# LPD-EPFL-ML/X-MAP

Hardware: NVIDIA B200
Metric: item_pair_sims_per_sec (higher is better)
Workload: dtype f64 epilogue over i64 fixed-point accumulators

## Files before the change

### include/xmap_b200.h

```cpp
#ifndef XMAP_B200_H
#define XMAP_B200_H

#include <stdbool.h>
#include <stddef.h>
#include <stdint.h>

#ifdef __cplusplus
extern "C" {
#endif

#define XMAP_B200_ABI_VERSION 8
#define XMAP_KMAX 64
#define XMAP_METHOD_ADJUST_COSINE 0
#define XMAP_METHOD_COSINE 1

int xmap_abi_version(void);
const char *xmap_last_error(void);

size_t xmap_layout_workspace_bytes(int64_t nnz, int32_t n_users, int32_t n_items);

int xmap_build_layout(const int32_t *user, const int32_t *item, const float *rating,
                      int64_t nnz, int32_t n_users, int32_t n_items,
                      int32_t *csr_ptr, uint64_t *csr_ent, int32_t *csr_src,
                      int32_t *csc_ptr, uint64_t *csc_ent,
                      double *user_mu, double *item_stats,
                      void *workspace, size_t workspace_bytes, void *stream);

int xmap_row_work(const int32_t *csr_ptr, const int32_t *csc_ptr, const uint64_t *csc_ent,
                  int32_t n_items, int64_t *row_work, void *stream);

size_t xmap_tri_workspace_bytes(int64_t nnz);
int xmap_build_tri_layout(const int32_t *csr_ptr, const uint64_t *csr_ent,
                          const int32_t *csc_ptr, const uint64_t *csc_ent,
                          const double *user_mu, const double *item_stats, const int32_t *prefix_code,
                          const int32_t *ord, int32_t n_users, int32_t n_items, int64_t nnz, int32_t method,
                          int32_t e_base, uint64_t *tcsr_ent, void *csc_aux, void *ostat, int64_t *tri_work,
                          void *workspace, size_t workspace_bytes, void *stream);

typedef struct xmap_sim_args {
    const int32_t *csc_ptr; const uint64_t *csc_ent; const void *csc_aux;
    const uint64_t *tcsr_ent;
    const void *ostat; const int32_t *ord; const int64_t *tri_work;
    const int32_t *ord_item;
    const uint8_t *dom_code;
    const uint8_t *contains;
    int32_t n_items; int32_t method; int32_t num_atleast; int32_t k;
    int32_t r2_bits;
    int32_t count_only;
    const int64_t *rec_ptr;
    int32_t *rec_cnt;
    void *rec;
    int32_t *rec_n;
    uint8_t *bb;
    int32_t *row_npairs;
    int32_t *tab_idx; double *tab_sim; int32_t *tab_mutu; int32_t *tab_n; int32_t *tab_len;
    int32_t *error_flag;
} xmap_sim_args;

#define XMAP_SIM_ROW_HDR_BYTES 48
int xmap_sim_row_headers(const xmap_sim_args *args_h, const int32_t *rows, int32_t n_rows,
                         const int32_t *seg_lo, const int32_t *seg_hi, void *hdr_out, void *stream);

#define XMAP_SIM_MAX_SMEM_CELLS 12288
int64_t xmap_sim_row_cells(int64_t tri_work, int32_t n_more_popular);
int xmap_sim_accumulate(const xmap_sim_args *args_h, const void *row_hdr, int32_t n_rows,
                        int32_t cells_cap, int32_t threads_per_row,
                        void *gtab, int32_t gtab_ctas, void *stream);

int xmap_sim_accumulate_split(const xmap_sim_args *args_h, const void *seg_hdr, const int32_t *seg_slot,
                              const int32_t *slot_nseg, int32_t n_segs, int32_t cells_cap, void *gtab,
                              int32_t *done, void *stream);

#define XMAP_SELECT_LONG 8192
int xmap_sim_select(const xmap_sim_args *args_h, const int32_t *rows, int32_t n_rows,
                    int32_t long_rows, void *stream);

int xmap_segmented_copy16(const void *src, const int64_t *src_pos, void *dst, const int64_t *dst_pos,
                          const int64_t *seg_off, int32_t n_seg, int64_t total, void *stream);
int xmap_segmented_copy4(const void *src, const int64_t *src_pos, void *dst, const int64_t *dst_pos,
                         const int64_t *seg_off, int32_t n_seg, int64_t total, void *stream);

#define XMAP_XSIM_MAX_CELLS_LG 13
typedef struct xmap_xsim_args {
    int32_t n_starts;
    int32_t n_units;
    const int32_t *unit_order;
    int32_t *unit_counter;
    int32_t warps;
    const int64_t *unit_leg_lo, *unit_leg_hi;
    const int32_t *unit_g0, *unit_g1;
    const int32_t *unit_npass;
    const int32_t *start_unit_ptr;
    const int64_t *lp_ptr;
    const int32_t *pd_s;
    const double *pd_n, *pd_d, *pd_c;
    const int64_t *rs_ptr;
    const int32_t *rs_end;
    const double *rs_n, *rs_d, *rs_c;
    const int32_t *tile_ptr; int32_t gb;
    int32_t cells_lg;
    const int32_t *unit_clg;
    void *gws; int32_t gcells_lg;
    int32_t top_m;
    int32_t merge;
    int32_t *unit_count; int64_t *unit_combos;
    int32_t *unit_top_end; double *unit_top_xsim; int32_t *unit_top_len;
    int32_t *out_count; int64_t *out_combos;
    int32_t *top_end; double *top_xsim; int32_t *top_len;
    const int64_t *emit_ptr; int32_t *emit_end; double *emit_xsim;
    int32_t *error_flag;
    int64_t *unit_cycles;
} xmap_xsim_args;

int64_t xmap_xsim_smem_bytes(int32_t cells_lg, int32_t warps);
int xmap_xsim_extend(const xmap_xsim_args *args_h, void *stream);
int64_t xmap_xsim_cta_smem_bytes(int32_t cells_lg);
int xmap_xsim_extend_cta(const xmap_xsim_args *args_h, void *stream);
int xmap_xsim_merge(const xmap_xsim_args *args_h, void *stream);

int xmap_choose_mapping(const int32_t *top_end, const double *top_xsim, const int32_t *top_len,
                        int32_t n_rows, int32_t top_m, int32_t mode, int32_t n_cand,
                        double epsilon, int32_t mapping_range, int32_t global_sensitivity,
                        const double *uniforms, uint64_t seed,
                        int32_t *chosen, void *stream);

int xmap_invert_mapping(const int32_t *start_item, const int32_t *chosen, int32_t n_rows,
                        int32_t *map, void *stream);

size_t xmap_alterego_workspace_bytes(int64_t nnz);
int xmap_build_alterego(const int32_t *csr_ptr, const uint64_t *csr_ent, const int32_t *csr_src,
                        const int64_t *ts, int32_t n_users, int64_t nnz, const int32_t *map,
                        int32_t *out_user, int32_t *out_item, double *out_rating, int64_t *out_ts,
                        int64_t *n_out_h, void *workspace, size_t workspace_bytes, void *stream);

int xmap_recsim_item_info(const int64_t *item_ptr, const double *rating_by_item, int32_t n_items, double *info,
                          void *stream);
int xmap_recsim_fill_entries(const int64_t *user_ptr, const int64_t *ent_off, int32_t n_users, const int32_t *item,
                             int64_t n_items, int64_t total, int64_t *key, int64_t *src, void *stream);
int xmap_recsim_pairs(const int64_t *seg_ptr, const int64_t *seg_key, const int64_t *src, const double *rating,
                      const double *info, int64_t n_items, int64_t n_pairs, int32_t num_atleast,
                      int32_t *out_i, int32_t *out_j, int64_t *out_n, double *out_sim, double *out_ls, void *stream);

int xmap_recsim_neighbors(const int64_t *row_ptr, const int32_t *pair_j, const double *pair_sim, int32_t n_items,
                          int32_t k, int32_t *nb_idx, double *nb_sim, int32_t *nb_len, void *stream);
int xmap_recsim_predict(const int64_t *prof_ptr, const int32_t *prof_item, const double *prof_rating,
                        const int64_t *prof_ts, const double *info, const int32_t *nb_idx, const double *nb_sim,
                        const int32_t *nb_len, int32_t k, const int32_t *t_user, const int32_t *t_item, int64_t n_test,
                        double alpha, double *pred_nodecay, double *pred_decay, int32_t *error_flag, void *stream);

int xmap_recsim_private_neighbor(const int64_t *row_ptr, const int32_t *nbr, const double *sim, const double *ls,
                                 int32_t n_items, int32_t mapping_range, double eps, double rpo,
                                 const double *u_pick, const double *u_noise, uint64_t seed, double *scratch,
                                 int32_t *out_nbr, double *out_sim, int32_t *out_len, void *stream);

int xmap_clean_records(const int32_t *user, const int32_t *item, const double *ts, const int64_t *order,
                       int64_t n, int32_t n_users, double t_lo, double t_hi, int32_t num_atleast,
                       uint8_t *keep, int32_t *user_items, void *stream);

#define XMAP_INGEST_ID_MAX 48
#define XMAP_INGEST_OK 0
#define XMAP_INGEST_BLANK 1
#define XMAP_INGEST_FEW_FIELDS 2
#define XMAP_INGEST_NON_ASCII 3
#define XMAP_INGEST_NUL 4
#define XMAP_INGEST_BAD_TIME 5
#define XMAP_INGEST_TIME_RANGE 6
#define XMAP_INGEST_BAD_RATING 7
#define XMAP_INGEST_UID_LONG 8
#define XMAP_INGEST_IID_LONG 9
int xmap_ingest_line_masks(const void *buf, int64_t size, uint16_t *masks, int32_t *block_cnt, void *stream);
int xmap_ingest_line_offsets(const uint16_t *masks, int64_t size, const int64_t *block_off, int64_t *offs, void *stream);
int xmap_ingest_parse(const uint8_t *buf, const int64_t *offs, int64_t n_lines, const char *label_h, int32_t label_len,
                      double ts_min, double ts_max, int64_t ld, uint8_t *status, double *rating, double *ts,
                      uint64_t *uid_words, uint8_t *uid_len, uint64_t *iid_words, uint8_t *iid_len, void *stream);
int xmap_ingest_rank_flags(const uint64_t *words, int64_t ld, int32_t n_words, const int64_t *perm, int64_t n,
                           int32_t *flag, void *stream);
int xmap_ingest_rank_scatter(const int64_t *perm, const int32_t *flag, const int64_t *csum, int64_t n, int32_t *rank,
                             int64_t *rep, void *stream);
int xmap_ingest_first(const int32_t *user, const int32_t *item, const double *ts, const int64_t *order,
                      const uint8_t *keep, int64_t n, double t_lo, double t_hi, int32_t *first_user, int32_t *pair_first,
                      void *stream);
int xmap_ingest_item_suffix(const uint64_t *iid_words, int64_t ld, const uint8_t *iid_len, const int64_t *rep,
                            int32_t n_items, uint8_t *present, void *stream);
int xmap_ingest_item_codes(const uint64_t *iid_words, int64_t ld, const uint8_t *iid_len, const int64_t *rep,
                           int32_t n_items, const int32_t *labels, int32_t n_labels, int32_t *prefix_new,
                           uint8_t *dom_code, uint8_t *contains, bool *has_S, bool *has_T, void *stream);
int xmap_ingest_train_keys(const int32_t *user, const int32_t *item, const int8_t *grp, const int32_t *upos,
                           const bool *has_S, const int32_t *srank, int64_t n, int64_t *key, void *stream);

#ifdef __cplusplus
}
#endif
#endif
```

### x-map_b200/csrc/sim.cu

```cuda
#include "common.cuh"

namespace xmap {

constexpr int KMAX = XMAP_KMAX;

struct __align__(16) OStat {
    double den;
    uint32_t item;
    uint32_t prefix_exp;
};

struct __align__(16) Cell {
    unsigned key, cnt, lo, hi;
};

struct __align__(16) Rec {
    unsigned long long sim;
    unsigned long long pack;
};
__device__ __forceinline__ unsigned long long rec_pack(unsigned item, unsigned mutu) {
    return (unsigned long long)item | ((unsigned long long)mutu << 32);
}
__device__ __forceinline__ int rec_item(unsigned long long p) { return int((unsigned)p); }
__device__ __forceinline__ int rec_mutu(unsigned long long p) { return int((unsigned)(p >> 32)); }

struct __align__(16) RowHdr {
    int row, oi, lo, hi;
    long long work;
    double den;
    long long rec_base;
    unsigned prefix_exp;
    int rec_cap;
};
static_assert(sizeof(RowHdr) == 48, "RowHdr layout");

__device__ __forceinline__ RowHdr load_hdr(const RowHdr *p) {
    const uint4 *q = reinterpret_cast<const uint4 *>(p);
    const uint4 a = __ldg(q), b = __ldg(q + 1), c = __ldg(q + 2);
    RowHdr h;
    h.row = (int)a.x; h.oi = (int)a.y; h.lo = (int)a.z; h.hi = (int)a.w;
    h.work = (long long)(((unsigned long long)b.y << 32) | b.x);
    h.den = __hiloint2double((int)b.w, (int)b.z);
    h.rec_base = (long long)(((unsigned long long)c.y << 32) | c.x);
    h.prefix_exp = c.z; h.rec_cap = (int)c.w;
    return h;
}

__global__ void row_headers_kernel(xmap_sim_args a, const int32_t *__restrict__ rows, int n_rows,
                                   const int32_t *__restrict__ seg_lo, const int32_t *__restrict__ seg_hi,
                                   RowHdr *__restrict__ out) {
    const int r = blockIdx.x * blockDim.x + threadIdx.x;
    if (r >= n_rows) return;
    const int row = rows[r];
    const OStat *ostat = reinterpret_cast<const OStat *>(a.ostat);
    RowHdr h;
    h.row = row; h.oi = a.ord[row];
    h.lo = seg_lo ? seg_lo[r] : a.csc_ptr[row];
    h.hi = seg_hi ? seg_hi[r] : a.csc_ptr[row + 1];
    h.work = a.tri_work[row];
    const OStat si = ostat[h.oi];
    h.den = si.den; h.prefix_exp = si.prefix_exp;
    h.rec_base = a.rec_ptr[row];
    h.rec_cap = (int)(a.rec_ptr[row + 1] - a.rec_ptr[row]);
    out[r] = h;
}

__host__ __device__ __forceinline__ long long hash_cells_for(long long work) {
    long long c = (work * 4 + 2) / 3;
    return c < 32 ? 32 : c;
}

template <bool CTA_ROW>
__device__ __forceinline__ void group_sync() {
    if (CTA_ROW) __syncthreads(); else __syncwarp();
}

struct RaterDesc {
    unsigned start;
    int len;
    double ci, mu;
};

__device__ __forceinline__ RaterDesc load_rater(const xmap_sim_args &a, int e, int hi) {
    RaterDesc d{0u, 0, 0.0, 0.0};
    if (e < hi) {
        const uint2 ce = ld_ent(a.csc_ent + e);
        const uint4 ax = __ldg(reinterpret_cast<const uint4 *>(a.csc_aux) + e);
        d.mu = __hiloint2double((int)ax.w, (int)ax.z);
        d.ci = (double)__uint_as_float(ce.y) - d.mu;
        d.start = (ax.x + 1u) | (ce.x & 0x80000000u);
        d.len = (int)ax.y;
    }
    return d;
}

struct SplitCtx {
    uint4 *gtab;
    int *done;
    int nseg;
};

template <bool CTA_ROW, class IDX>
__device__ void tri_row(const xmap_sim_args &a, Cell *__restrict__ T, IDX *__restrict__ occ_list, int *s_cnt,
                        int cells_cap, const RowHdr *hdr_p, const SplitCtx *sp = nullptr) {
    const int lane = threadIdx.x & 31;
    const int gwarps = CTA_ROW ? (blockDim.x >> 5) : 1;
    const int gw = CTA_ROW ? (threadIdx.x >> 5) : 0;
    const int gthreads = gwarps * 32, gtid = gw * 32 + lane;
    const unsigned lt_mask = (1u << lane) - 1u;
    const OStat *__restrict__ ostat = reinterpret_cast<const OStat *>(a.ostat);

    const RowHdr hd = load_hdr(hdr_p);
    const int row = hd.row, oi = hd.oi;
    const int e_i = int(hd.prefix_exp & 0xFFu);
    const unsigned prefix_i = hd.prefix_exp >> 8;
    const int lo = hd.lo, hi = hd.hi;
    const long long work = hd.work;
    const int rtop = a.n_items - 1 - oi;
    const long long hcells = hash_cells_for(work);
    const bool direct = (long long)rtop <= hcells;
    const long long ncell_ll = direct ? (long long)rtop : hcells;
    if (ncell_ll > cells_cap || (!direct && min((long long)(hi - lo), work) >= 65536)) {
        if (gtid == 0) atomicExch(a.error_flag, ncell_ll > cells_cap ? 1 : 3);
        return;
    }
    const int ncell = (int)ncell_ll;
    uint4 *T4 = reinterpret_cast<uint4 *>(T);
    for (int s = gtid; s < ncell; s += gthreads) T4[s] = make_uint4(0u, 0u, 0u, 0u);
    if (CTA_ROW && gtid == 0) *s_cnt = 0;
    group_sync<CTA_ROW>();

    const int qbase = 62 - a.r2_bits;
    const int top_ord = a.n_items - 1;
    const bool coop = CTA_ROW && ((hi - lo + 31) >> 5) < gwarps;
    const int bfirst = coop ? 0 : gw, bstride = coop ? 1 : gwarps;
    const int cfirst = coop ? gw : 0, cstride = coop ? gwarps : 1;
    constexpr int UC = 2;
    RaterDesc nxt = load_rater(a, lo + bfirst * 32 + lane, hi);
    for (int b0 = lo + bfirst * 32; b0 < hi; b0 += bstride * 32) {
        const RaterDesc cur = nxt;
        nxt = load_rater(a, b0 + bstride * 32 + lane, hi);
        int incl = cur.len;
#pragma unroll
        for (int off = 1; off < 32; off <<= 1) {
            const int t = __shfl_up_sync(0xffffffffu, incl, off);
            if (lane >= off) incl += t;
        }
        const int total = __shfl_sync(0xffffffffu, incl, 31);
        const int excl = incl - cur.len;
        for (int t0 = cfirst * 32; t0 < total; t0 += cstride * 32 * UC) {
            uint2 en[UC];
            unsigned st_l[UC];
            double ci_l[UC], mu_l[UC];
            bool valid[UC];
#pragma unroll
            for (int u = 0; u < UC; ++u) {
                const int t = t0 + u * cstride * 32 + lane;
                int l = 0;
#pragma unroll
                for (int step = 16; step >= 1; step >>= 1) {
                    const int v = __shfl_sync(0xffffffffu, incl, l + step - 1);
                    if (v <= t) l += step;
                }
                st_l[u] = __shfl_sync(0xffffffffu, cur.start, l);
                const int ex_l = __shfl_sync(0xffffffffu, excl, l);
                ci_l[u] = __shfl_sync(0xffffffffu, cur.ci, l);
                mu_l[u] = __shfl_sync(0xffffffffu, cur.mu, l);
                valid[u] = t < total;
                if (valid[u]) en[u] = ld_ent(a.tcsr_ent + ((st_l[u] & 0x7FFFFFFFu) + (unsigned)(t - ex_l)));
            }
#pragma unroll
            for (int u = 0; u < UC; ++u) {
                if (!valid[u]) continue;
                const int oj = ent_item(en[u].x);
                const double cj = (double)__uint_as_float(en[u].y) - mu_l[u];
                const double p = __dmul_rn(ci_l[u], cj);
                const int q = qbase - (e_i + ent_exp(en[u].x));
                const long long fx = __double2ll_rn(p * pow2d(q));
                const unsigned agree = ((unsigned)ent_ge(en[u].x) == (st_l[u] >> 31)) ? 1u : 0u;
                int slot;
                bool ok = true;
                if (direct) {
                    slot = top_ord - oj;
                    atomicAdd(agree ? &T[slot].key : &T[slot].cnt, 1u);
                } else {
                    const unsigned key = (unsigned)oj + 1u;
                    slot = (int)__umulhi((unsigned)oj * 2654435761u, (unsigned)ncell);
                    ok = false;
                    for (int probe = 0; probe < ncell; ++probe) {
                        unsigned c = *(volatile unsigned *)&T[slot].key;
                        if (c != key) {
                            if (c == 0u) c = atomicCAS(&T[slot].key, 0u, key);
                            if (c != 0u && c != key) { slot = (slot + 1 == ncell) ? 0 : slot + 1; continue; }
                        }
                        ok = true;
                        break;
                    }
                    if (ok) atomicAdd(&T[slot].cnt, (1u << 16) | agree);
                    else atomicExch(a.error_flag, 1);
                }
                if (ok) {
                    if (sizeof(IDX) == 4) {
                        atomicAdd(reinterpret_cast<unsigned long long *>(&T[slot].lo), (unsigned long long)fx);
                    } else {
                        const unsigned flo = (unsigned)(unsigned long long)fx;
                        unsigned fhi = (unsigned)((unsigned long long)fx >> 32);
                        if (flo) {
                            const unsigned old = atomicAdd(&T[slot].lo, flo);
                            fhi += ((unsigned)(old + flo) < old) ? 1u : 0u;
                        }
                        if (fhi) atomicAdd(&T[slot].hi, fhi);
                    }
                }
            }
        }
    }
    group_sync<CTA_ROW>();

    if (CTA_ROW && sp) {
        if (!direct) {
            if (gtid == 0) atomicExch(a.error_flag, 1);
            return;
        }
        for (int s = gtid; s < ncell; s += gthreads) {
            const uint4 v = T4[s];
            if (v.x) atomicAdd(&sp->gtab[s].x, v.x);
            if (v.y) atomicAdd(&sp->gtab[s].y, v.y);
            const unsigned long long fx = ((unsigned long long)v.w << 32) | v.z;
            if (fx) atomicAdd(reinterpret_cast<unsigned long long *>(&sp->gtab[s].z), fx);
        }
        __threadfence();
        __syncthreads();
        if (gtid == 0) *s_cnt = (atomicAdd(sp->done, 1) == sp->nseg - 1) ? 1 : 0;
        __syncthreads();
        const bool last = *s_cnt != 0;
        __syncthreads();
        if (!last) return;
        __threadfence();
        for (int s = gtid; s < ncell; s += gthreads) {
            T4[s] = __ldcg(sp->gtab + s);
            sp->gtab[s] = make_uint4(0u, 0u, 0u, 0u);
        }
        if (gtid == 0) { *sp->done = 0; *s_cnt = 0; }
        __syncthreads();
    }

    int n_ent = 0;
    for (int s0 = gw * 32; s0 < ncell; s0 += gthreads) {
        const int s = s0 + lane;
        bool occ = false;
        if (s < ncell) {
            const uint2 kc = *reinterpret_cast<const uint2 *>(&T[s]);
            occ = direct ? (kc.x | kc.y) != 0u : kc.x != 0u;
        }
        const unsigned m = __ballot_sync(0xffffffffu, occ);
        if (m) {
            int base = n_ent;
            if (CTA_ROW) {
                if (lane == 0) base = atomicAdd(s_cnt, __popc(m));
                base = __shfl_sync(0xffffffffu, base, 0);
            }
            if (occ) occ_list[base + __popc(m & lt_mask)] = (IDX)s;
            n_ent += __popc(m);
        }
    }
    group_sync<CTA_ROW>();
    if (CTA_ROW) n_ent = *s_cnt;
    if (gtid == 0 && n_ent) a.row_npairs[row] += n_ent;

    constexpr int EU = 2;
    int nkept = 0;
    for (int i0 = gtid; i0 < n_ent; i0 += gthreads * EU) {
        uint4 cv[EU];
        int sidx[EU];
        unsigned n[EU], mutu[EU];
        OStat sj[EU];
#pragma unroll
        for (int u = 0; u < EU; ++u) {
            const int i = i0 + u * gthreads;
            sidx[u] = -1;
            if (i < n_ent) {
                sidx[u] = (int)occ_list[i];
                cv[u] = T4[sidx[u]];
                int oj;
                if (direct) { n[u] = cv[u].x + cv[u].y; mutu[u] = cv[u].x; oj = top_ord - sidx[u]; }
                else { oj = (int)cv[u].x - 1; n[u] = cv[u].y >> 16; mutu[u] = cv[u].y & 0xFFFFu; }
                sj[u] = ostat[oj];
            }
        }
#pragma unroll
        for (int u = 0; u < EU; ++u) {
            if (sidx[u] < 0) continue;
            uint4 out = make_uint4(0u, 0u, 0u, 0u);
            const int q = qbase - (e_i + int(sj[u].prefix_exp & 0xFFu));
            const long long fx = (long long)(((unsigned long long)cv[u].w << 32) | (unsigned long long)cv[u].z);
            if (fx == 0 || mutu[u] == 0u) { T4[sidx[u]] = out; continue; }
            const double inner = (double)fx * pow2d(-q);
            const double dd = __dmul_rn(hd.den, sj[u].den);
            const double cosv = (dd != 0.0) ? __ddiv_rn(inner, dd) : 0.0;
            const int mn = min((int)n[u], a.num_atleast);
            const double sim = __ddiv_rn(__dmul_rn(cosv, (double)mn), (double)a.num_atleast);
            if (sim != 0.0 && mutu[u] != 0u) {
                ++nkept;
                const unsigned long long sb = (unsigned long long)__double_as_longlong(sim);
                out = direct ? make_uint4(mutu[u], n[u], (unsigned)sb, (unsigned)(sb >> 32))
                             : make_uint4(sj[u].item, (n[u] << 16) | mutu[u], (unsigned)sb, (unsigned)(sb >> 32));
                if ((sj[u].prefix_exp >> 8) != prefix_i) { a.bb[row] = 1; a.bb[sj[u].item] = 1; }
            }
            T4[sidx[u]] = out;
        }
    }
#pragma unroll
    for (int off = 16; off > 0; off >>= 1) nkept += __shfl_xor_sync(0xffffffffu, nkept, off);
    if (nkept == 0) return;

    Rec *__restrict__ rec = reinterpret_cast<Rec *>(a.rec);
    const long long base_i = hd.rec_base;
    const int cap_i = hd.rec_cap;
    int wbase = 0;
    if (lane == 0) wbase = atomicAdd(a.rec_cnt + row, nkept);
    wbase = __shfl_sync(0xffffffffu, wbase, 0);
    if (a.count_only) {
        for (int i = gw * 32 + lane; i < n_ent; i += gthreads) {
            const int sl = (int)occ_list[i];
            const uint4 cv = T4[sl];
            if ((cv.z | cv.w) != 0u) atomicAdd(a.rec_cnt + (direct ? __ldg(a.ord_item + (top_ord - sl)) : (int)cv.x), 1);
        }
        return;
    }
    if (wbase + nkept > cap_i) {
        if (lane == 0) atomicExch(a.error_flag, 2);
        return;
    }
    for (int i0 = gw * 32; i0 < n_ent; i0 += gthreads * EU) {
        uint4 cv[EU];
        bool keep[EU];
        long long base_j[EU];
        int cap_j[EU], p2[EU], jit[EU];
        unsigned nn[EU], mu[EU];
#pragma unroll
        for (int u = 0; u < EU; ++u) {
            const int i = i0 + u * gthreads + lane;
            int sl = 0;
            cv[u] = make_uint4(0u, 0u, 0u, 0u);
            if (i < n_ent) { sl = (int)occ_list[i]; cv[u] = T4[sl]; }
            keep[u] = (cv[u].z | cv[u].w) != 0u;
            jit[u] = 0; nn[u] = mu[u] = 0u;
            if (keep[u]) {
                if (direct) { jit[u] = __ldg(a.ord_item + (top_ord - sl)); mu[u] = cv[u].x; nn[u] = cv[u].y; }
                else { jit[u] = (int)cv[u].x; nn[u] = cv[u].y >> 16; mu[u] = cv[u].y & 0xFFFFu; }
            }
        }
#pragma unroll
        for (int u = 0; u < EU; ++u) {
            if (keep[u]) {
                base_j[u] = a.rec_ptr[jit[u]];
                cap_j[u] = (int)(a.rec_ptr[jit[u] + 1] - base_j[u]);
                p2[u] = atomicAdd(a.rec_cnt + jit[u], 1);
            }
        }
#pragma unroll
        for (int u = 0; u < EU; ++u) {
            const unsigned m = __ballot_sync(0xffffffffu, keep[u]);
            if (keep[u]) {
                const unsigned long long sb = ((unsigned long long)cv[u].w << 32) | cv[u].z;
// ... 397 lines not shown
            got = rr + 1;
        }
        if (lane == 0) {
            S.t_len[list] = got;
            S.thr[list] = (got == K) ? (last_k & ABS_MASK) : 0ull;
        }
    }
    __syncthreads();
    if (tid == 0) S.ncand = 0;
    __syncthreads();
}

constexpr int FIN_THREADS = 256;
constexpr int SEL_UNROLL = 4;
constexpr int SEL_CAP = 12 * FIN_THREADS;

__global__ void __launch_bounds__(FIN_THREADS) select_cta_kernel(xmap_sim_args a, const int32_t *__restrict__ rows,
                                                                 int n_rows) {
    extern __shared__ __align__(16) unsigned char smem_raw[];
    using ScratchT = Scratch<FIN_THREADS, SEL_CAP>;
    ScratchT &S = *reinterpret_cast<ScratchT *>(smem_raw);
    const int tid = threadIdx.x;
    const int row = rows ? rows[blockIdx.x] : blockIdx.x;
    const int m = a.rec_cnt[row];
    if (m <= XMAP_SELECT_LONG) return;
    const Rec *__restrict__ R = reinterpret_cast<const Rec *>(a.rec) + a.rec_ptr[row];
    const int32_t *__restrict__ RN = a.rec_n + a.rec_ptr[row];
    const bool bb_i = a.bb[row] != 0;
    const int dom_i = a.dom_code[row];
    const int K = a.k;
    if (tid == 0) {
        S.ncand = 0;
        S.t_len[0] = S.t_len[1] = 0; S.thr[0] = S.thr[1] = 0ull;
    }
    __syncthreads();
    for (int base = 0; base < m; base += FIN_THREADS * SEL_UNROLL) {
        if (S.ncand + 2 * FIN_THREADS * SEL_UNROLL + 2 * KMAX > SEL_CAP) select_lists<FIN_THREADS, SEL_CAP>(S, K);
        const unsigned long long f0 = S.thr[0], f1 = S.thr[1];
        const unsigned long long floor_key = (f0 < f1) ? f0 : f1;
        Rec v[SEL_UNROLL];
#pragma unroll
        for (int u = 0; u < SEL_UNROLL; ++u) {
            const int e = base + u * FIN_THREADS + tid;
            v[u] = (e < m) ? R[e] : Rec{0ull, 0ull};
        }
#pragma unroll
        for (int u = 0; u < SEL_UNROLL; ++u) {
            if (v[u].sim == 0ull) continue;
            const unsigned long long key = v[u].sim & ABS_MASK;
            if (key < floor_key) continue;
            const int j = rec_item(v[u].pack);
            const unsigned lb = list_bits(a, bb_i, dom_i, j);
#pragma unroll
            for (int lst = 0; lst < 2; ++lst) {
                if (!((lb >> lst) & 1u)) continue;
                const unsigned long long th = lst == 0 ? f0 : f1;
                if (th && key < th) continue;
                const int p = atomicAdd(&S.ncand, 1);
                S.skey[p] = (lst == 0 ? LIST0_BIT : 0ull) | key;
                S.spay[p] = (v[u].sim & LIST0_BIT) | ((unsigned long long)j << 16) | (unsigned)p;
                S.c_mutu[p] = rec_mutu(v[u].pack); S.c_n[p] = RN[base + u * FIN_THREADS + tid];
            }
        }
        __syncthreads();
    }
    select_lists<FIN_THREADS, SEL_CAP>(S, K);
    for (int slot = 0; slot < 2; ++slot) {
        const int len = S.t_len[slot];
        const size_t o = ((size_t)row * 2 + slot) * K;
        if (tid < len) {
            a.tab_idx[o + tid] = S.t_j[slot][tid]; a.tab_sim[o + tid] = S.t_sim[slot][tid];
            a.tab_mutu[o + tid] = S.t_mutu[slot][tid]; a.tab_n[o + tid] = S.t_n[slot][tid];
        }
        if (tid == 0) a.tab_len[(size_t)row * 2 + slot] = len;
    }
}

static int check_args(const xmap_sim_args &a) {
    if (a.k < 1 || a.k > KMAX) return fail_msg("xmap_sim: k out of range [1, XMAP_KMAX]");
    if (a.method != XMAP_METHOD_ADJUST_COSINE && a.method != XMAP_METHOD_COSINE)
        return fail_msg("xmap_sim: bad method");
    if (a.num_atleast < 1) return fail_msg("xmap_sim: num_atleast must be >= 1");
    return 0;
}

}

using namespace xmap;

extern "C" int64_t xmap_sim_row_cells(int64_t tri_work, int32_t n_more_popular) {
    const long long h = hash_cells_for(tri_work);
    return (long long)n_more_popular <= h ? (long long)n_more_popular : h;
}

extern "C" int xmap_sim_row_headers(const xmap_sim_args *args_h, const int32_t *rows, int32_t n_rows,
                                    const int32_t *seg_lo, const int32_t *seg_hi, void *hdr_out, void *stream_) {
    if (n_rows <= 0) return 0;
    cudaStream_t st = (cudaStream_t)stream_;
    row_headers_kernel<<<(n_rows + 255) / 256, 256, 0, st>>>(*args_h, rows, n_rows, seg_lo, seg_hi,
                                                             reinterpret_cast<RowHdr *>(hdr_out));
    XMAP_LAUNCH_CHECK();
    return 0;
}

extern "C" int xmap_sim_accumulate(const xmap_sim_args *args_h, const void *hdr_, int32_t n_rows,
                                   int32_t cells_cap, int32_t threads_per_row,
                                   void *gtab, int32_t gtab_ctas, void *stream_) {
    const RowHdr *rows = reinterpret_cast<const RowHdr *>(hdr_);
    if (int rc = check_args(*args_h)) return rc;
    if (n_rows <= 0) return 0;
    cudaStream_t st = (cudaStream_t)stream_;
    if (threads_per_row < 32 || threads_per_row > 512 || (threads_per_row & 31))
        return fail_msg("xmap_sim_accumulate: threads_per_row must be a multiple of 32 in [32, 512]");
    if (cells_cap < 1) return fail_msg("xmap_sim_accumulate: cells_cap must be positive");
    if (gtab) {
        if (gtab_ctas < 1) return fail_msg("xmap_sim_accumulate: gtab_ctas must be positive");
        const int grid = n_rows < gtab_ctas ? n_rows : gtab_ctas;
        tri_gmem_kernel<<<grid, threads_per_row < 64 ? 64 : threads_per_row, 0, st>>>(
            *args_h, rows, n_rows, cells_cap, reinterpret_cast<unsigned char *>(gtab));
        XMAP_LAUNCH_CHECK();
        return 0;
    }
    if (cells_cap > XMAP_SIM_MAX_SMEM_CELLS) return fail_msg("xmap_sim_accumulate: cells_cap exceeds shared memory");
    if (threads_per_row == 32) {
        const size_t smem = 4 * row_smem_bytes(cells_cap);
        if (smem > 227 * 1024) return fail_msg("xmap_sim_accumulate: warp-row tables exceed shared memory");
        XMAP_CUDA(cudaFuncSetAttribute(tri_warp_kernel, cudaFuncAttributeMaxDynamicSharedMemorySize, (int)smem));
        tri_warp_kernel<<<(n_rows + 3) / 4, 128, smem, st>>>(*args_h, rows, n_rows, cells_cap);
    } else {
        const size_t smem = row_smem_bytes(cells_cap);
        XMAP_CUDA(cudaFuncSetAttribute(tri_cta_kernel, cudaFuncAttributeMaxDynamicSharedMemorySize, (int)smem));
        tri_cta_kernel<<<n_rows, threads_per_row, smem, st>>>(*args_h, rows, n_rows, cells_cap);
    }
    XMAP_LAUNCH_CHECK();
    return 0;
}

extern "C" int xmap_sim_accumulate_split(const xmap_sim_args *args_h, const void *hdr_, const int32_t *seg_slot,
                                         const int32_t *slot_nseg, int32_t n_segs, int32_t cells_cap, void *gtab,
                                         int32_t *done, void *stream_) {
    if (int rc = check_args(*args_h)) return rc;
    if (n_segs <= 0) return 0;
    if (cells_cap < 1 || cells_cap > XMAP_SIM_MAX_SMEM_CELLS)
        return fail_msg("xmap_sim_accumulate_split: cells_cap out of range");
    cudaStream_t st = (cudaStream_t)stream_;
    const size_t smem = row_smem_bytes(cells_cap);
    XMAP_CUDA(cudaFuncSetAttribute(tri_split_kernel, cudaFuncAttributeMaxDynamicSharedMemorySize, (int)smem));
    tri_split_kernel<<<n_segs, 512, smem, st>>>(*args_h, reinterpret_cast<const RowHdr *>(hdr_), seg_slot, slot_nseg,
                                                cells_cap, reinterpret_cast<uint4 *>(gtab), done);
    XMAP_LAUNCH_CHECK();
    return 0;
}

extern "C" int xmap_sim_select(const xmap_sim_args *args_h, const int32_t *rows, int32_t n_rows,
                               int32_t long_rows, void *stream_) {
    if (int rc = check_args(*args_h)) return rc;
    if (n_rows <= 0) return 0;
    cudaStream_t st = (cudaStream_t)stream_;
    if (!long_rows) {
        select_warp_kernel<<<(n_rows + 3) / 4, 128, 0, st>>>(*args_h, rows, n_rows);
    } else {
        const size_t sel_smem = sizeof(Scratch<FIN_THREADS, SEL_CAP>);
        XMAP_CUDA(cudaFuncSetAttribute(select_cta_kernel, cudaFuncAttributeMaxDynamicSharedMemorySize, (int)sel_smem));
        select_cta_kernel<<<n_rows, FIN_THREADS, sel_smem, st>>>(*args_h, rows, n_rows);
    }
    XMAP_LAUNCH_CHECK();
    return 0;
}
```

### x-map_b200/engine.py

```python
import os
from dataclasses import dataclass, field

import torch

from . import _native as N



def _stream_ptr():
    return torch.cuda.current_stream().cuda_stream


def _dev(t, dtype, device):
    return torch.as_tensor(t, dtype=dtype).to(device, non_blocking=True).contiguous()


@dataclass
class ItemMeta:
    prefix_code: torch.Tensor
    dom_code: torch.Tensor
    contains: torch.Tensor
    has_S: torch.Tensor
    has_T: torch.Tensor


def to_device_meta(meta, device="cuda"):
    T = lambda key, dt: torch.as_tensor(meta[key], dtype=dt, device=device)
    return ItemMeta(prefix_code=T("prefix_code", torch.int32), dom_code=T("dom_code", torch.uint8),
                    contains=T("contains", torch.uint8), has_S=T("has_S", torch.bool), has_T=T("has_T", torch.bool))


@dataclass
class Layout:
    n_users: int
    n_items: int
    nnz: int
    csr_ptr: torch.Tensor
    csr_ent: torch.Tensor
    csr_src: torch.Tensor
    csc_ptr: torch.Tensor
    csc_ent: torch.Tensor
    user_mu: torch.Tensor
    item_stats: torch.Tensor
    row_work: torch.Tensor


def build_layout(user, item, rating, n_users, n_items, device="cuda"):
    L = N.lib()
    user = _dev(user, torch.int32, device)
    item = _dev(item, torch.int32, device)
    rating = _dev(rating, torch.float32, device)
    nnz = int(user.numel())
    i32 = dict(dtype=torch.int32, device=device)
    f64 = dict(dtype=torch.float64, device=device)
    csr_ptr = torch.empty(n_users + 1, **i32)
    csc_ptr = torch.empty(n_items + 1, **i32)
    csr_ent = torch.empty(nnz, dtype=torch.int64, device=device)
    csc_ent = torch.empty(nnz, dtype=torch.int64, device=device)
    csr_src = torch.empty(nnz, **i32)
    user_mu = torch.empty(n_users, **f64)
    item_stats = torch.empty(n_items, 4, **f64)
    ws_bytes = L.xmap_layout_workspace_bytes(nnz, n_users, n_items)
    ws = torch.empty(ws_bytes, dtype=torch.uint8, device=device)
    N.check(L.xmap_build_layout(N.ptr(user), N.ptr(item), N.ptr(rating), nnz, n_users, n_items,
                                N.ptr(csr_ptr), N.ptr(csr_ent), N.ptr(csr_src),
                                N.ptr(csc_ptr), N.ptr(csc_ent), N.ptr(user_mu), N.ptr(item_stats),
                                N.ptr(ws), ws_bytes, _stream_ptr()), "xmap_build_layout")
    row_work = torch.empty(n_items, dtype=torch.int64, device=device)
    N.check(L.xmap_row_work(N.ptr(csr_ptr), N.ptr(csc_ptr), N.ptr(csc_ent), n_items,
                            N.ptr(row_work), _stream_ptr()), "xmap_row_work")
    del ws
    return Layout(n_users, n_items, nnz, csr_ptr, csr_ent, csr_src, csc_ptr, csc_ent,
                  user_mu, item_stats, row_work)


EXP_FIELD_MAX = 127
EXP_CLAMP_MAX = 16


def exponent_base(method, item_stats):
    den = item_stats[:, 1 if method == "cosine" else 2]
    den = den[den > 0]
    if den.numel() == 0:
        return 0
    e = torch.frexp(den).exponent
    lo, hi = int(e.min()), int(e.max())
    if hi - lo > EXP_FIELD_MAX + EXP_CLAMP_MAX:
        raise ValueError("item norms span 2^%d (from 2^%d to 2^%d): more than the similarity stage's fixed-point "
                         "inner product resolves (2^%d)" % (hi - lo, lo - 1, hi, EXP_FIELD_MAX + EXP_CLAMP_MAX))
    return hi - EXP_FIELD_MAX


@dataclass
class SimTables:
    k: int
    n_items: int
    row_flags: torch.Tensor
    row_npairs: torch.Tensor
    row_nkept: torch.Tensor
    tab_idx: torch.Tensor
    tab_sim: torch.Tensor
    tab_mutu: torch.Tensor
    tab_n: torch.Tensor
    tab_len: torch.Tensor
    launches: int = 0
    stats: dict = field(default_factory=dict)

    @property
    def n_pairs_total(self):
        return 2 * int(self.row_npairs.sum().item())


CELL_CLASSES = tuple(int(c) for c in os.environ.get("XMAP_CELL_CLASSES", "256,512,1024,1536,2048,3072,4096,6144,8192,12288").split(","))


def _threads_for_cells(c):
    return max(32, min(512, (c // 8 + 31) // 32 * 32))

REC_BYTES = 20
SPLIT_RATERS = int(os.environ.get("XMAP_SPLIT_RATERS", "16384"))
SPLIT_SEG = 4096
_PINNED = {}


_REC_POOL = {}


def _rec_words(n_records):
    n = max(int(n_records), 1)
    return 2 * n + (n + 1) // 2


def _rec_buffer(n_records, device):
    need = _rec_words(n_records)
    pool = _REC_POOL.setdefault(str(device), [])
    fit = [q for q, t in enumerate(pool) if t.numel() >= need]
    if fit:
        return pool.pop(min(fit, key=lambda q: pool[q].numel()))
    pool.clear()
    return torch.empty(need, dtype=torch.int64, device=device)


def _rec_views(raw, n_records):
    n = max(int(n_records), 1)
    return raw[:2 * n].view(n, 2), raw[2 * n:2 * n + (n + 1) // 2].view(torch.int32)[:n]


def popularity_order(count):
    I = int(count.numel())
    key = count.long() * (1 << 24) + torch.arange(I, device=count.device)
    perm = torch.argsort(key)
    ord_ = torch.empty(I, dtype=torch.int32, device=count.device)
    ord_[perm] = torch.arange(I, dtype=torch.int32, device=count.device)
    return ord_


class SimEngine:

    def __init__(self, layout, meta, method="adjust_cosine", num_atleast=50, k=10,
                 max_smem_cells=CELL_CLASSES[-1], rec_budget=None):
        if method not in N.METHODS:
            raise ValueError("unknown similarity method %r" % (method,))
        if not (1 <= k <= N.KMAX):
            raise ValueError("top_k must be in [1, %d]" % N.KMAX)
        self.lay, self.meta = layout, meta
        self.method, self.num_atleast, self.k = method, int(num_atleast), int(k)
        self.device = layout.csr_ptr.device
        self.e_base = exponent_base(method, layout.item_stats)
        self.max_smem_cells = int(max_smem_cells)
        self.launches = 0
        I = layout.n_items
        dev = self.device
        L = N.lib()
        count = layout.item_stats[:, 3]
        self.ord = popularity_order(count)
        self.ord_item = torch.empty(I, dtype=torch.int32, device=dev)
        self.ord_item[self.ord.long()] = torch.arange(I, dtype=torch.int32, device=dev)
        self.tcsr_ent = torch.empty(layout.nnz, dtype=torch.int64, device=dev)
        self.csc_aux = torch.empty((layout.nnz, 2), dtype=torch.int64, device=dev)
        self.ostat = torch.empty(max(I, 1) * 16, dtype=torch.uint8, device=dev)
        self.tri_work = torch.zeros(I, dtype=torch.int64, device=dev)
        ws_bytes = L.xmap_tri_workspace_bytes(layout.nnz)
        ws = torch.empty(ws_bytes, dtype=torch.uint8, device=dev)
        N.check(L.xmap_build_tri_layout(
            N.ptr(layout.csr_ptr), N.ptr(layout.csr_ent), N.ptr(layout.csc_ptr), N.ptr(layout.csc_ent),
            N.ptr(layout.user_mu), N.ptr(layout.item_stats), N.ptr(meta.prefix_code), N.ptr(self.ord),
            layout.n_users, I, layout.nnz, N.METHODS[method], self.e_base,
            N.ptr(self.tcsr_ent), N.ptr(self.csc_aux), N.ptr(self.ostat), N.ptr(self.tri_work),
            N.ptr(ws), ws_bytes, _stream_ptr()), "xmap_build_tri_layout")
        del ws
        cap = torch.clamp(layout.row_work - count.long(), min=0, max=max(I - 1, 0))
        self.rec_ptr = torch.zeros(I + 1, dtype=torch.int64, device=dev)
        self.rec_ptr[1:] = torch.cumsum(cap, 0)
        self.rec_cap = cap
        self.rec_cap_bound = cap
        total = int(self.rec_ptr[-1].item()) if I else 0
        if rec_budget is None:
            free, _ = torch.cuda.mem_get_info(dev)
            pooled = max((t.numel() * 8 for t in _REC_POOL.get(str(dev), [])), default=0)
            rec_budget = max(free // 2, pooled)
        self.exact_sizing = total * REC_BYTES > rec_budget
        self._rec_raw = None
        self.rec = self.rec_n = None
        if not self.exact_sizing:
            self._set_rec(_rec_buffer(total, dev), total)
        self.rec_cnt = torch.zeros(I, dtype=torch.int32, device=dev)
        self.bb = torch.zeros(I, dtype=torch.uint8, device=dev)
        self.row_npairs = torch.zeros(I, dtype=torch.int32, device=dev)
        self.error_flag = torch.zeros(1, dtype=torch.int32, device=dev)
        self.tab_idx = torch.full((I, 2, k), -1, dtype=torch.int32, device=dev)
        self.tab_sim = torch.zeros((I, 2, k), dtype=torch.float64, device=dev)
        self.tab_mutu = torch.zeros((I, 2, k), dtype=torch.int32, device=dev)
        self.tab_n = torch.zeros((I, 2, k), dtype=torch.int32, device=dev)
        self.tab_len = torch.zeros((I, 2), dtype=torch.int32, device=dev)
        self._gtab = None
        self._side = None
        self._plans = {}
        self.profile = None

    def _set_rec(self, raw, n_records):
        self._rec_raw = raw
        self.rec, self.rec_n = _rec_views(raw, n_records)

    def _give_back(self):
        raw = getattr(self, "_rec_raw", None)
        self._rec_raw = self.rec = self.rec_n = None
        if raw is not None and raw.numel() > (1 << 21) and _REC_POOL is not None:
            pool = _REC_POOL.setdefault(str(raw.device), [])
            if len(pool) < 2:
                pool.append(raw)

    def __del__(self):
        try:
            self._give_back()
        except Exception:
            pass

    def release_lists(self):
        self._give_back()
        self.exact_sizing = True

    def _args(self):
        lay, m = self.lay, self.meta
        a = N.SimArgs()
        a.csc_ptr, a.csc_ent, a.csc_aux = N.ptr(lay.csc_ptr), N.ptr(lay.csc_ent), N.ptr(self.csc_aux)
        a.tcsr_ent = N.ptr(self.tcsr_ent)
        a.ostat, a.ord, a.tri_work = N.ptr(self.ostat), N.ptr(self.ord), N.ptr(self.tri_work)
        a.ord_item = N.ptr(self.ord_item)
        a.dom_code, a.contains = N.ptr(m.dom_code), N.ptr(m.contains)
        a.n_items, a.method = lay.n_items, N.METHODS[self.method]
        a.num_atleast, a.k, a.r2_bits = self.num_atleast, self.k, 2 * self.e_base
        a.rec_ptr, a.rec_cnt, a.rec, a.rec_n = N.ptr(self.rec_ptr), N.ptr(self.rec_cnt), N.ptr(self.rec), N.ptr(self.rec_n)
        a.count_only = 1 if self.rec is None else 0
        a.bb, a.row_npairs = N.ptr(self.bb), N.ptr(self.row_npairs)
        a.tab_idx, a.tab_sim = N.ptr(self.tab_idx), N.ptr(self.tab_sim)
        a.tab_mutu, a.tab_n, a.tab_len = N.ptr(self.tab_mutu), N.ptr(self.tab_n), N.ptr(self.tab_len)
        a.error_flag = N.ptr(self.error_flag)
        return a

    def plan(self, rows=None):
        key = None
        if rows is not None:
            n = int(rows.numel())
            lo = int(rows[0]) if n else -1
            contiguous = n == 0 or (int(rows[-1]) == lo + n - 1 and bool((rows[1:] - rows[:-1] == 1).all()))
            key = (lo, n) if contiguous else ("set", hash(tuple(rows.cpu().tolist())))
        if key in self._plans:
            return self._plans[key]
        dev, I = self.device, self.lay.n_items
        if rows is None:
            rows = torch.arange(I, dtype=torch.int32, device=dev)
        else:
            rows = rows.to(dev, dtype=torch.int32)
        rl = rows.long()
        work = self.tri_work[rl]
        rtop = (I - 1 - self.ord[rl]).long()
        h = torch.clamp((work * 4 + 2) // 3, min=32)
        cells = torch.where(rtop <= h, rtop, h)
        classes = [c for c in CELL_CLASSES if c <= self.max_smem_cells] or [self.max_smem_cells]
        if classes[-1] < self.max_smem_cells:
            classes.append(self.max_smem_cells)
        bounds = torch.tensor(classes, dtype=torch.int64, device=dev)
        cls = torch.bucketize(cells, bounds)
        t_cells = torch.tensor([_threads_for_cells(c) for c in classes] + [512], dtype=torch.int64, device=dev)[cls]
        t_work = torch.full_like(work, 32)
        t_work[work > 3072] = 128
        t_work[work > 8192] = 256
        t_work[work > 32768] = 512
        threads = torch.maximum(t_cells, t_work)
        live = work > 0
        craters = (self.lay.csc_ptr[rl + 1] - self.lay.csc_ptr[rl]).long()
        is_split = live & (rtop <= h) & (craters >= SPLIT_RATERS) & (cells <= self.max_smem_cells)
        split = None
        if bool(is_split.any()):
            srows, sr_c = rows[is_split], craters[is_split]
            o = torch.argsort(sr_c, descending=True, stable=True)
            srows, sr_c = srows[o], sr_c[o]
            nseg = (sr_c + SPLIT_SEG - 1) // SPLIT_SEG
            slot = torch.repeat_interleave(torch.arange(srows.numel(), device=dev), nseg)
            q = torch.arange(int(nseg.sum().item()), device=dev) - (torch.cumsum(nseg, 0) - nseg)[slot]
            base = self.lay.csc_ptr[srows.long()].long()[slot]
            seg_lo = base + q * SPLIT_SEG
            seg_hi = torch.minimum(seg_lo + SPLIT_SEG, base + sr_c[slot])
            cap = max(32, int(cells[is_split].max().item()))
            i32 = lambda t: t.to(torch.int32).contiguous()
            split = dict(hdr=self._headers(i32(srows[slot]), i32(seg_lo), i32(seg_hi)), seg_slot=i32(slot),
                         slot_nseg=i32(nseg), n_segs=int(slot.numel()), cells_cap=cap, rows=srows,
                         gtab=torch.zeros((srows.numel() * cap, 2), dtype=torch.int64, device=dev),
                         done=torch.zeros(srows.numel(), dtype=torch.int32, device=dev))
            live = live & ~is_split
        code = (cls * 2048 + threads)[live]
        rows_l, work_l, cells_l = rows[live], work[live], cells[live]
        order = torch.argsort(code * (1 << 40) + ((1 << 40) - 1 - work_l.clamp(max=(1 << 40) - 1)))
        rows_s = rows_l[order].contiguous()
        codes, counts = torch.unique_consecutive(code[order], return_counts=True)
        gmax = torch.zeros(int(cls.max().item()) * 2048 + 2048 if cls.numel() else 1, dtype=torch.int64, device=dev)
        gmax.scatter_reduce_(0, code, cells_l, "amax")
        launches, at = [], 0
        for c, n, mx in zip(codes.tolist(), counts.tolist(), gmax[codes].tolist()):
            r = rows_s[at:at + n]
            at += n
            q, th = c // 2048, c % 2048
            if q < len(classes):
                launches.append((r, classes[q], th, False, self._headers(r)))
            else:
                launches.append((r, int(mx), 512, True, self._headers(r)))
        launches.sort(key=lambda t: (-t[2], -t[1]))
        long_cand = rows[self.rec_cap[rl] > N.SELECT_LONG].contiguous()
        out = (launches, long_cand, split)
        self._plans[key] = out
        return out

    def _headers(self, rows, seg_lo=None, seg_hi=None):
        n = int(rows.numel())
        hdr = torch.empty(max(n, 1) * N.ROW_HDR_BYTES, dtype=torch.uint8, device=self.device)
        N.check(N.lib().xmap_sim_row_headers(self._args(), N.ptr(rows), n, N.ptr(seg_lo), N.ptr(seg_hi), N.ptr(hdr),
                                             _stream_ptr()), "xmap_sim_row_headers")
        return hdr

    def enable_profile(self):
        self.profile = {}

    def _timed(self, kind, fn):
        if self.profile is None:
            return fn()
        a, b = torch.cuda.Event(enable_timing=True), torch.cuda.Event(enable_timing=True)
        a.record()
        r = fn()
        b.record()
        self.profile.setdefault(kind, []).append((a, b))
        return r

    def profile_ms(self):
        torch.cuda.synchronize()
        out = {k: (len(v), sum(a.elapsed_time(b) for a, b in v)) for k, v in (self.profile or {}).items()}
        self.profile = {}
        return out

    def _check_error(self):
        e = int(self.error_flag.item())
        if e != 0:
            raise N.NativeError("similarity kernel error %d (1: table overflow, 2: record-list capacity, "
                                "3: co-rating count out of range)" % e)

    def reset(self):
        self.rec_cnt.zero_()
        self.bb.zero_()
        self.row_npairs.zero_()

    def _size_lists(self, rows=None):
        self._give_back()
        self.reset()
        self._accumulate(rows)
        self._check_error()
        return self.rec_cnt.long().clone()

    def _alloc_lists(self, lengths):
        I, dev = self.lay.n_items, self.device
        self.rec_ptr = torch.zeros(I + 1, dtype=torch.int64, device=dev)
        self.rec_ptr[1:] = torch.cumsum(lengths, 0)
        self.rec_cap = lengths
        total = int(self.rec_ptr[-1].item()) if I else 0
        self._set_rec(_rec_buffer(total, dev), total)
        self._plans = {}
        self.reset()

    def accumulate(self, rows=None):
        if self.rec is None:
            self._alloc_lists(self._size_lists(rows))
        return self._accumulate(rows)

    def _accumulate(self, rows=None):
        L = N.lib()
        args = self._args()
        launches, _, split = self.plan(rows)
        main = torch.cuda.current_stream()
        n_streams = int(os.environ.get("XMAP_SIM_STREAMS", "3"))
        use_side = self.profile is None and len(launches) > 1 and n_streams > 1
        if use_side and self._side is None:
            self._side = [torch.cuda.Stream(device=self.device) for _ in range(n_streams - 1)]
        if use_side:
            for sd in self._side:
                sd.wait_stream(main)
        stats = []
        if split is not None:
            sp = split
            self._timed("accumulate_split", lambda: N.check(L.xmap_sim_accumulate_split(
                args, N.ptr(sp["hdr"]), N.ptr(sp["seg_slot"]), N.ptr(sp["slot_nseg"]), sp["n_segs"], sp["cells_cap"],
                N.ptr(sp["gtab"]), N.ptr(sp["done"]), main.cuda_stream), "xmap_sim_accumulate_split"))
            self.launches += 1
            stats.append(("accumulate_split", int(sp["rows"].numel())))
        for q, (r, cells_cap, threads, in_gmem, hdr) in enumerate(launches):
            gtab, ctas = None, 0
            if in_gmem:
                ctas = min(int(r.numel()), 296)
                need = ctas * ((cells_cap * 20 + 15) // 16 * 16)
                if self._gtab is None or self._gtab.numel() < need:
                    self._gtab = None
                    self._gtab = torch.empty(need, dtype=torch.uint8, device=self.device)
                gtab = self._gtab
            kind = "accumulate_%s%d_t%d" % ("g" if in_gmem else "c", cells_cap, threads)
            stream = main
            if use_side and not in_gmem and q % n_streams:
                stream = self._side[q % n_streams - 1]
            st = stream.cuda_stream
            self._timed(kind, lambda: N.check(L.xmap_sim_accumulate(
                args, N.ptr(hdr), r.numel(), cells_cap, threads, N.ptr(gtab), ctas, st), "xmap_sim_accumulate"))
            self.launches += 1
            stats.append((kind, int(r.numel())))
        if use_side:
            for sd in self._side:
                main.wait_stream(sd)
        return stats

    def select(self, rows=None):
        L = N.lib()
        st = _stream_ptr()
        args = self._args()
        _, long_cand, _ = self.plan(rows)
        n = self.lay.n_items if rows is None else int(rows.numel())
        rp = None if rows is None else N.ptr(rows.to(self.device, dtype=torch.int32).contiguous())
        self._timed("select_warp", lambda: N.check(L.xmap_sim_select(args, rp, n, 0, st), "xmap_sim_select"))
# ... 60 lines not shown
```

Measured before the change: 23.27 billion.

## Replace shared-memory atomics with warp-owned cell updates for warp-per-row hashing

For rows handled by a single warp, the hash/direct cell update now uses a claim-and-own scheme instead of atomics. Each lane writes its lane id into a claim array keyed by slot, and the winning lane does a plain 128-bit read-modify-write. After a few rounds, any lanes still pending fall back to the old atomic path. Small-work rows also get a sparser hash table (2x instead of 4/3), which should shorten probe chains, at the cost of more shared memory per row. The change also adds optional stats counters, and it reuses occ_list as the claim buffer, which depends on that buffer being large enough.

Result: faster. 23.89 billion (median of 6 runs) (+2.6%).

```diff
diff --git a/include/xmap_b200.h b/include/xmap_b200.h
--- a/include/xmap_b200.h
+++ b/include/xmap_b200.h
@@ -62,6 +62,7 @@
                          const int32_t *seg_lo, const int32_t *seg_hi, void *hdr_out, void *stream);
 
 #define XMAP_SIM_MAX_SMEM_CELLS 12288
+#define XMAP_SIM_SMALL_HASH_WORK 2048
 int64_t xmap_sim_row_cells(int64_t tri_work, int32_t n_more_popular);
 int xmap_sim_accumulate(const xmap_sim_args *args_h, const void *row_hdr, int32_t n_rows,
                         int32_t cells_cap, int32_t threads_per_row,
diff --git a/x-map_b200/csrc/sim.cu b/x-map_b200/csrc/sim.cu
--- a/x-map_b200/csrc/sim.cu
+++ b/x-map_b200/csrc/sim.cu
@@ -66,7 +66,7 @@
 }
 
 __host__ __device__ __forceinline__ long long hash_cells_for(long long work) {
-    long long c = (work * 4 + 2) / 3;
+    long long c = work <= XMAP_SIM_SMALL_HASH_WORK ? work * 2 : (work * 4 + 2) / 3;
     return c < 32 ? 32 : c;
 }
 
@@ -99,6 +99,104 @@
     int *done;
     int nseg;
 };
+
+#ifdef XMAP_SIM_OWN_STATS
+__device__ unsigned long long g_own_stats[3];
+#endif
+
+template <bool GMEM>
+__device__ __forceinline__ void cell_add_atomic(Cell *__restrict__ T, int *error_flag, bool direct, int ncell,
+                                                int top_ord, int oj, unsigned agree, long long fx) {
+    int slot;
+    bool ok = true;
+    if (direct) {
+        slot = top_ord - oj;
+        atomicAdd(agree ? &T[slot].key : &T[slot].cnt, 1u);
+    } else {
+        const unsigned key = (unsigned)oj + 1u;
+        slot = (int)__umulhi((unsigned)oj * 2654435761u, (unsigned)ncell);
+        ok = false;
+        for (int probe = 0; probe < ncell; ++probe) {
+            unsigned c = *(volatile unsigned *)&T[slot].key;
+            if (c != key) {
+                if (c == 0u) c = atomicCAS(&T[slot].key, 0u, key);
+                if (c != 0u && c != key) { slot = (slot + 1 == ncell) ? 0 : slot + 1; continue; }
+            }
+            ok = true;
+            break;
+        }
+        if (ok) atomicAdd(&T[slot].cnt, (1u << 16) | agree);
+        else atomicExch(error_flag, 1);
+    }
+    if (ok) {
+        if (GMEM) {
+            atomicAdd(reinterpret_cast<unsigned long long *>(&T[slot].lo), (unsigned long long)fx);
+        } else {
+            const unsigned flo = (unsigned)(unsigned long long)fx;
+            unsigned fhi = (unsigned)((unsigned long long)fx >> 32);
+            if (flo) {
+                const unsigned old = atomicAdd(&T[slot].lo, flo);
+                fhi += ((unsigned)(old + flo) < old) ? 1u : 0u;
+            }
+            if (fhi) atomicAdd(&T[slot].hi, fhi);
+        }
+    }
+}
+
+constexpr int OWN_ROUNDS = 3;
+
+__device__ __forceinline__ void cell_add_owned(Cell *__restrict__ T, unsigned short *__restrict__ claim,
+                                               int *error_flag, bool direct, int ncell, int top_ord, int oj,
+                                               unsigned agree, long long fx, bool pend, int lane) {
+    uint4 *T4 = reinterpret_cast<uint4 *>(T);
+    const unsigned key = (unsigned)oj + 1u;
+    int slot = direct ? top_ord - oj : (int)__umulhi((unsigned)oj * 2654435761u, (unsigned)ncell);
+    int probes = 0;
+#ifdef XMAP_SIM_OWN_STATS
+    int rounds = 0;
+    const bool any = __any_sync(0xffffffffu, pend);
+#endif
+#pragma unroll 1
+    for (int round = 0; round < OWN_ROUNDS; ++round) {
+        if (!__any_sync(0xffffffffu, pend)) break;
+#ifdef XMAP_SIM_OWN_STATS
+        ++rounds;
+#endif
+        if (pend && !direct) {
+            unsigned c = T[slot].key;
+            while (c != key && c != 0u) {
+                if (++probes >= ncell) break;
+                slot = (slot + 1 == ncell) ? 0 : slot + 1;
+                c = T[slot].key;
+            }
+            if (probes >= ncell) { atomicExch(error_flag, 1); pend = false; }
+        }
+        if (pend) claim[slot] = (unsigned short)lane;
+        __syncwarp();
+        if (pend && claim[slot] == (unsigned short)lane) {
+            uint4 v = T4[slot];
+            if (direct) { v.x += agree; v.y += agree ^ 1u; }
+            else { v.x = key; v.y += (1u << 16) | agree; }
+            const unsigned long long s = (((unsigned long long)v.w << 32) | v.z) + (unsigned long long)fx;
+            v.z = (unsigned)s; v.w = (unsigned)(s >> 32);
+            T4[slot] = v;
+            pend = false;
+        }
+        __syncwarp();
+    }
+    const unsigned left = __ballot_sync(0xffffffffu, pend);
+#ifdef XMAP_SIM_OWN_STATS
+    if (lane == 0 && any) {
+        atomicAdd(&g_own_stats[0], 1ull);
+        atomicAdd(&g_own_stats[1], (unsigned long long)rounds);
+        atomicAdd(&g_own_stats[2], (unsigned long long)__popc(left));
+    }
+#endif
+    if (left) {
+        if (pend) cell_add_atomic<false>(T, error_flag, direct, ncell, top_ord, oj, agree, fx);
+        __syncwarp();
+    }
+}
 
 template <bool CTA_ROW, class IDX>
 __device__ void tri_row(const xmap_sim_args &a, Cell *__restrict__ T, IDX *__restrict__ occ_list, int *s_cnt,
@@ -171,46 +269,22 @@
             }
 #pragma unroll
             for (int u = 0; u < UC; ++u) {
-                if (!valid[u]) continue;
-                const int oj = ent_item(en[u].x);
-                const double cj = (double)__uint_as_float(en[u].y) - mu_l[u];
-                const double p = __dmul_rn(ci_l[u], cj);
-                const int q = qbase - (e_i + ent_exp(en[u].x));
-                const long long fx = __double2ll_rn(p * pow2d(q));
-                const unsigned agree = ((unsigned)ent_ge(en[u].x) == (st_l[u] >> 31)) ? 1u : 0u;
-                int slot;
-                bool ok = true;
-                if (direct) {
-                    slot = top_ord - oj;
-                    atomicAdd(agree ? &T[slot].key : &T[slot].cnt, 1u);
-                } else {
-                    const unsigned key = (unsigned)oj + 1u;
-                    slot = (int)__umulhi((unsigned)oj * 2654435761u, (unsigned)ncell);
-                    ok = false;
-                    for (int probe = 0; probe < ncell; ++probe) {
-                        unsigned c = *(volatile unsigned *)&T[slot].key;
-                        if (c != key) {
-                            if (c == 0u) c = atomicCAS(&T[slot].key, 0u, key);
-                            if (c != 0u && c != key) { slot = (slot + 1 == ncell) ? 0 : slot + 1; continue; }
-                        }
-                        ok = true;
-                        break;
-                    }
-                    if (ok) atomicAdd(&T[slot].cnt, (1u << 16) | agree);
-                    else atomicExch(a.error_flag, 1);
+                int oj = 0;
+                long long fx = 0;
+                unsigned agree = 0u;
+                if (valid[u]) {
+                    oj = ent_item(en[u].x);
+                    const double cj = (double)__uint_as_float(en[u].y) - mu_l[u];
+                    const double p = __dmul_rn(ci_l[u], cj);
+                    const int q = qbase - (e_i + ent_exp(en[u].x));
+                    fx = __double2ll_rn(p * pow2d(q));
+                    agree = ((unsigned)ent_ge(en[u].x) == (st_l[u] >> 31)) ? 1u : 0u;
                 }
-                if (ok) {
-                    if (sizeof(IDX) == 4) {
-                        atomicAdd(reinterpret_cast<unsigned long long *>(&T[slot].lo), (unsigned long long)fx);
-                    } else {
-                        const unsigned flo = (unsigned)(unsigned long long)fx;
-                        unsigned fhi = (unsigned)((unsigned long long)fx >> 32);
-                        if (flo) {
-                            const unsigned old = atomicAdd(&T[slot].lo, flo);
-                            fhi += ((unsigned)(old + flo) < old) ? 1u : 0u;
-                        }
-                        if (fhi) atomicAdd(&T[slot].hi, fhi);
-                    }
+                if (!CTA_ROW) {
+                    cell_add_owned(T, reinterpret_cast<unsigned short *>(occ_list), a.error_flag, direct, ncell,
+                                   top_ord, oj, agree, fx, valid[u], lane);
+                } else if (valid[u]) {
+                    cell_add_atomic<sizeof(IDX) == 4>(T, a.error_flag, direct, ncell, top_ord, oj, agree, fx);
                 }
             }
         }
@@ -914,6 +988,16 @@
     return 0;
 }
 
+#ifdef XMAP_SIM_OWN_STATS
+extern "C" int xmap_sim_own_stats(unsigned long long *out3) {
+    XMAP_CUDA(cudaDeviceSynchronize());
+    XMAP_CUDA(cudaMemcpyFromSymbol(out3, g_own_stats, sizeof(g_own_stats)));
+    const unsigned long long zero[3] = {0ull, 0ull, 0ull};
+    XMAP_CUDA(cudaMemcpyToSymbol(g_own_stats, zero, sizeof(zero)));
+    return 0;
+}
+#endif
+
 extern "C" int xmap_sim_select(const xmap_sim_args *args_h, const int32_t *rows, int32_t n_rows,
                                int32_t long_rows, void *stream_) {
     if (int rc = check_args(*args_h)) return rc;
diff --git a/x-map_b200/engine.py b/x-map_b200/engine.py
--- a/x-map_b200/engine.py
+++ b/x-map_b200/engine.py
@@ -117,6 +117,10 @@
 def _threads_for_cells(c):
     return max(32, min(512, (c // 8 + 31) // 32 * 32))
 
+
+WARP_ROW_THREADS = int(os.environ.get("XMAP_WARP_ROW_THREADS", "32"))
+
+SMALL_HASH_WORK = 2048
 REC_BYTES = 20
 SPLIT_RATERS = int(os.environ.get("XMAP_SPLIT_RATERS", "16384"))
 SPLIT_SEG = 4096
@@ -275,7 +279,7 @@
         rl = rows.long()
         work = self.tri_work[rl]
         rtop = (I - 1 - self.ord[rl]).long()
-        h = torch.clamp((work * 4 + 2) // 3, min=32)
+        h = torch.clamp(torch.where(work <= SMALL_HASH_WORK, work * 2, (work * 4 + 2) // 3), min=32)
         cells = torch.where(rtop <= h, rtop, h)
         classes = [c for c in CELL_CLASSES if c <= self.max_smem_cells] or [self.max_smem_cells]
         if classes[-1] < self.max_smem_cells:
@@ -288,6 +292,7 @@
         t_work[work > 8192] = 256
         t_work[work > 32768] = 512
         threads = torch.maximum(t_cells, t_work)
+        threads[(t_work == 32) & (t_cells <= WARP_ROW_THREADS)] = 32
         live = work > 0
         craters = (self.lay.csc_ptr[rl + 1] - self.lay.csc_ptr[rl]).long()
         is_split = live & (rtop <= h) & (craters >= SPLIT_RATERS) & (cells <= self.max_smem_cells)
```
